# hyye/lio-mapping

Hardware: AMD Instinct MI355X
Metric: sliding-window solves/sec, 64-line 130k-pt scans, window=15 (opt_window=5) (higher is better)
Workload: dtype f64 (solve) / f32 (features); 1 GPU; HDL-64E outdoor_test_config_64, S_outdoor ray-cast scans, window_size=15 opt_window_size=5, one SolveOptimization per step, clouds resident in HBM; n_lidar_residuals=78236, local_map_points=76752, surf_stack_points=19386, parallelism=1 window

## Files before the change

lio-mapping_amd/csrc/cloud_device.h:

```cpp
#pragma once
#include <hip/hip_runtime.h>

#include <cfloat>
#include <climits>

#include "cloud_kernels.h"
#include "hmath.h"

#if defined(__HIPCC__)
namespace lio {

__device__ inline bool finite3(const float4 &p) { return isfinite(p.x) && isfinite(p.y) && isfinite(p.z); }
__device__ inline bool finite3(const Vec3<float> &p) { return isfinite(p.x) && isfinite(p.y) && isfinite(p.z); }


template <bool NORMALISE_CONJ>
__device__ __forceinline__ float4 to_end_point(float4 p, float s, const Quat<float> &qe, const Vec3<float> &te) {
  p.x -= s * te.x; p.y -= s * te.y; p.z -= s * te.z;
  Quat<float> qid;
  Quat<float> qs = slerp(qid, s, qe, FLT_EPSILON);
  Quat<float> qc = conj(qs);
  if (NORMALISE_CONJ) qc = normalized(qc);
  Vec3<float> v = rotate(qc, Vec3<float>(p.x, p.y, p.z));
  v = rotate(qe, v);
  p.x = v.x + te.x; p.y = v.y + te.y; p.z = v.z + te.z;
  return p;
}
__device__ __forceinline__ float4 rigid_map_point(float4 p, const Quat<float> &q, const Vec3<float> &t) {
  const Vec3<float> v = rotate(q, Vec3<float>(p.x, p.y, p.z));
  return make_float4(v.x + t.x, v.y + t.y, v.z + t.z, p.w);
}

__device__ inline int cell_coord(float v, float inv_cell) { return int(floorf(v * inv_cell)); }
__device__ __forceinline__ bool cell_of(float x, float y, float z, const GridDesc &g, int &cx, int &cy, int &cz) {
  cx = cell_coord(x, g.inv_cell) - g.origin[0];
  cy = cell_coord(y, g.inv_cell) - g.origin[1];
  cz = cell_coord(z, g.inv_cell) - g.origin[2];
  return cx >= 0 && cy >= 0 && cz >= 0 && cx < g.dims[0] && cy < g.dims[1] && cz < g.dims[2];
}
__device__ __forceinline__ uint32_t cell_index(int cx, int cy, int cz, const GridDesc &g) { return uint32_t(cx + g.dims[0] * (cy + g.dims[1] * cz)); }
__device__ __forceinline__ uint32_t cell_key_clamped(const float4 &p, const GridDesc &g) {
  int cx, cy, cz;
  cell_of(p.x, p.y, p.z, g, cx, cy, cz);
  cx = min(max(cx, 0), g.dims[0] - 1); cy = min(max(cy, 0), g.dims[1] - 1); cz = min(max(cz, 0), g.dims[2] - 1);
  return cell_index(cx, cy, cz, g);
}

__device__ __forceinline__ void cell_count_point(const float4 *__restrict__ pts, int i, const GridDesc &g, uint32_t *__restrict__ keys,
                                                 uint32_t *__restrict__ slot, int *__restrict__ cnt) {
  const uint32_t c = cell_key_clamped(pts[i], g);
  keys[i] = c;
  slot[i] = uint32_t(atomicAdd(&cnt[c], 1));
}
__device__ __forceinline__ void cell_place_point(const float4 *__restrict__ pts, const uint32_t *__restrict__ keys, const uint32_t *__restrict__ slot, int i,
                                                 const int *__restrict__ starts, float4 *__restrict__ sorted, int *__restrict__ cnt) {
  float4 p = pts[i];
  p.w = __int_as_float(i);
  const uint32_t c = keys[i];
  sorted[starts[c] + int(slot[i])] = p;
  cnt[c] = 0;
}

#define SEG_SCAN_THREADS 1024
#define SEG_SCAN_ITEMS 4
__device__ __forceinline__ void block_exclusive_scan(const int *__restrict__ in, int *__restrict__ out, int n, int base) {
  __shared__ int wsum[SEG_SCAN_THREADS / 64];
  const int tid = threadIdx.x, lane = tid & 63, wv = tid >> 6;
  int carry = base;
  for (int c0 = 0; c0 < n; c0 += SEG_SCAN_THREADS * SEG_SCAN_ITEMS) {
    const int i0 = c0 + tid * SEG_SCAN_ITEMS;
    int v[SEG_SCAN_ITEMS], tsum = 0;
#pragma unroll
    for (int k = 0; k < SEG_SCAN_ITEMS; ++k) { v[k] = i0 + k < n ? in[i0 + k] : 0; tsum += v[k]; }
    int inc = tsum;
#pragma unroll
    for (int off = 1; off < 64; off <<= 1) {
      const int u = __shfl_up(inc, off, 64);
      if (lane >= off) inc += u;
    }
    if (lane == 63) wsum[wv] = inc;
    __syncthreads();
    int before = 0, total = 0;
#pragma unroll
    for (int w = 0; w < SEG_SCAN_THREADS / 64; ++w) { const int t = wsum[w]; if (w < wv) before += t; total += t; }
    int run = carry + before + inc - tsum;
#pragma unroll
    for (int k = 0; k < SEG_SCAN_ITEMS; ++k)
      if (i0 + k < n) { out[i0 + k] = run; run += v[k]; }
    carry += total;
    __syncthreads();
  }
}

#define VOX_TILE 256
#define VOX_KEY_NONE 0xFFFFFFFFu

template <int ZBITS>
__device__ __forceinline__ bool vox_abs_key(const float4 &p, float inv_leaf, uint32_t &key) {
  constexpr int ZOFF = 1 << (ZBITS - 1);
  const float cx = floorf(p.x * inv_leaf), cy = floorf(p.y * inv_leaf), cz = floorf(p.z * inv_leaf);
  if (!(fabsf(cx) < 1024.f && fabsf(cy) < 1024.f && fabsf(cz) < float(ZOFF - 1))) return false;
  key = (uint32_t(int(cz) + ZOFF) << 22) | (uint32_t(int(cy) + 1024) << 11) | uint32_t(int(cx) + 1024);
  return true;
}

__device__ __forceinline__ void vox_block_partial(float (&mn)[3], float (&mx)[3], float cnt, float *__restrict__ row) {
  __shared__ float sm[7][VOX_TILE / 64];
  const int lane = threadIdx.x & 63, wv = threadIdx.x >> 6;
#pragma unroll
  for (int o = 32; o > 0; o >>= 1) {
    for (int d = 0; d < 3; ++d) { mn[d] = fminf(mn[d], __shfl_xor(mn[d], o, 64)); mx[d] = fmaxf(mx[d], __shfl_xor(mx[d], o, 64)); }
    cnt += __shfl_xor(cnt, o, 64);
  }
  if (lane == 0) { for (int d = 0; d < 3; ++d) { sm[d][wv] = mn[d]; sm[3 + d][wv] = mx[d]; } sm[6][wv] = cnt; }
  __syncthreads();
  if (threadIdx.x < 7) {
    const int t = threadIdx.x;
    float v = sm[t][0];
    for (int w = 1; w < VOX_TILE / 64; ++w) v = t < 3 ? fminf(v, sm[t][w]) : (t < 6 ? fmaxf(v, sm[t][w]) : v + sm[t][w]);
    row[t] = v;
  }
}

__device__ __forceinline__ bool vox_fold_bounds(const float *__restrict__ partial, int nb, float inv_leaf, VoxParams &v) {
  __shared__ float sm[7][VOX_TILE];
  const int t = threadIdx.x;
  float mn[3] = {FLT_MAX, FLT_MAX, FLT_MAX}, mx[3] = {-FLT_MAX, -FLT_MAX, -FLT_MAX};
  float cnt = 0;
  for (int b = t; b < nb; b += VOX_TILE) {
    for (int d = 0; d < 3; ++d) { mn[d] = fminf(mn[d], partial[size_t(b) * 8 + d]); mx[d] = fmaxf(mx[d], partial[size_t(b) * 8 + 3 + d]); }
    cnt += partial[size_t(b) * 8 + 6];
  }
  for (int d = 0; d < 3; ++d) { sm[d][t] = mn[d]; sm[3 + d][t] = mx[d]; }
  sm[6][t] = cnt;
  __syncthreads();
  for (int st = VOX_TILE / 2; st > 0; st >>= 1) {
    if (t < st) {
      for (int d = 0; d < 3; ++d) { sm[d][t] = fminf(sm[d][t], sm[d][t + st]); sm[3 + d][t] = fmaxf(sm[3 + d][t], sm[3 + d][t + st]); }
      sm[6][t] += sm[6][t + st];
    }
    __syncthreads();
  }
  if (t != 0) return false;
  long long dd[3];
  for (int d = 0; d < 3; ++d) {
    v.mn[d] = sm[d][0]; v.mx[d] = sm[3 + d][0];
    dd[d] = (long long)((v.mx[d] - v.mn[d]) * inv_leaf) + 1;
    v.minb[d] = int(floorf(v.mn[d] * inv_leaf));
    const int maxb = int(floorf(v.mx[d] * inv_leaf));
    v.divb[d] = maxb - v.minb[d] + 1;
  }
  v.overflow = (sm[6][0] > 0 && dd[0] * dd[1] * dd[2] > (long long)INT_MAX) ? 1 : 0;
  v.n_valid = int(sm[6][0]);
  return true;
}

__device__ __forceinline__ bool vox_is_head(const uint32_t *__restrict__ keys, int i, uint32_t k) {
  return k != VOX_KEY_NONE && (i == 0 || keys[i - 1] != k);
}
__device__ __forceinline__ void vox_tile_head_count(const uint32_t *__restrict__ keys, int n, int tile, int *__restrict__ count) {
  __shared__ int swave[VOX_TILE / 64];
  const int i = tile * VOX_TILE + threadIdx.x;
  const uint32_t k = i < n ? keys[i] : VOX_KEY_NONE;
  const unsigned long long b = __ballot(vox_is_head(keys, i, k));
  if ((threadIdx.x & 63) == 0) swave[threadIdx.x >> 6] = __popcll(b);
  __syncthreads();
  if (threadIdx.x == 0) *count = (swave[0] + swave[1]) + (swave[2] + swave[3]);
}

struct VoxSlot { int pos; bool head; };
__device__ __forceinline__ VoxSlot vox_centroid_tile(const float4 *__restrict__ pts, const uint32_t *__restrict__ keys, const uint32_t *__restrict__ vals,
                                                     const int *__restrict__ tile_heads, int n, int tile, float4 *__restrict__ out) {
  __shared__ float4 sp[VOX_TILE];
  __shared__ uint32_t sk[VOX_TILE];
  __shared__ int swave[VOX_TILE / 64], sbase[VOX_TILE / 64];
  const int tid = threadIdx.x, lane = tid & 63, wv = tid >> 6;
  const int base_i = tile * VOX_TILE, i = base_i + tid;
  int before = 0;
  for (int b = tid; b < tile; b += VOX_TILE) before += tile_heads[b];
#pragma unroll
  for (int o = 32; o > 0; o >>= 1) before += __shfl_xor(before, o, 64);
  const uint32_t k = i < n ? keys[i] : VOX_KEY_NONE;
  sk[tid] = k;
  if (k != VOX_KEY_NONE) sp[tid] = pts[vals[i]];
  const bool head = vox_is_head(keys, i, k);
  const unsigned long long hb = __ballot(head);
  if (lane == 0) { swave[wv] = __popcll(hb); sbase[wv] = before; }
  __syncthreads();
  int pos = (sbase[0] + sbase[1]) + (sbase[2] + sbase[3]);
  for (int w = 0; w < wv; ++w) pos += swave[w];
  pos += __popcll(hb & ((1ull << lane) - 1ull));
  if (head) {
    float ax = 0, ay = 0, az = 0, ai = 0;
    int e = tid;
    while (e < VOX_TILE && sk[e] == k) { const float4 p = sp[e]; ax += p.x; ay += p.y; az += p.z; ai += p.w; ++e; }
    int cnt = e - tid;
    if (e == VOX_TILE) {
      int g = base_i + VOX_TILE;
      while (g < n && keys[g] == k) { const float4 p = pts[vals[g]]; ax += p.x; ay += p.y; az += p.z; ai += p.w; ++g; ++cnt; }
    }
    const float c = float(cnt);
    out[pos] = make_float4(ax / c, ay / c, az / c, ai / c);
  }
  return VoxSlot{pos, head};
}

__device__ __forceinline__ void clear_valid_block(uint8_t *__restrict__ valid, size_t n) {
  const size_t i = (size_t(blockIdx.x) * VOX_TILE + threadIdx.x) * 16;
  if (i + 16 <= n) *reinterpret_cast<uint4 *>(valid + i) = make_uint4(0, 0, 0, 0);
  else for (size_t k = i; k < n; ++k) valid[k] = 0;
}
__device__ __forceinline__ void odom_state_init(OdomState *__restrict__ st, const float *__restrict__ T, bool converged) {
  static_assert(offsetof(OdomState, T) == 0 && sizeof(OdomState) <= VOX_TILE * 4, "state layout: T first, the rest zero");
  unsigned *o = reinterpret_cast<unsigned *>(st);
  const int nw = int(sizeof(OdomState) / 4);
  if (int(threadIdx.x) < nw) {
    unsigned v = threadIdx.x < 8 ? __float_as_uint(T[threadIdx.x]) : 0u;
    if (converged && threadIdx.x == offsetof(OdomState, converged) / 4) v = 1u;
    o[threadIdx.x] = v;
  }
}


#define FEAT_LPQ 8
#ifndef KNN_BATCH
#define KNN_BATCH 4
#endif
__device__ __forceinline__ unsigned long long knn_key(float d, int idx) {
  return (static_cast<unsigned long long>(__float_as_uint(d)) << 32) | static_cast<unsigned int>(idx);
}
template <int K>
__device__ __forceinline__ void knn_insert(unsigned long long key, int j, unsigned long long (&bk)[K], int (&bj)[K]) {
  if (key < bk[K - 1]) {
    bk[K - 1] = key; bj[K - 1] = j;
#pragma unroll
    for (int k = K - 1; k > 0; --k) {
      const bool sw = bk[k - 1] > bk[k];
      const unsigned long long tk = sw ? bk[k - 1] : bk[k];
      const int tj = sw ? bj[k - 1] : bj[k];
      bk[k - 1] = sw ? bk[k] : bk[k - 1];
      bj[k - 1] = sw ? bj[k] : bj[k - 1];
      bk[k] = tk; bj[k] = tj;
    }
  }
}
template <int K, int LPQ>
__device__ inline void knn_scan_group(const Vec3<float> &q, bool active, int sub, const float4 *__restrict__ map,
                                      const int *__restrict__ cells, const GridDesc &g, float (&bd)[K], int (&bi)[K], int (&bj)[K]) {
  unsigned long long bk[K];
#pragma unroll
  for (int k = 0; k < K; ++k) { bk[k] = knn_key(INFINITY, INT_MAX); bj[k] = 0; }
  int cx, cy, cz;
  cell_of(q.x, q.y, q.z, g, cx, cy, cz);
  if (!finite3(q) || cx < 0 || cy < 0 || cz < 0 || cx >= g.dims[0] || cy >= g.dims[1] || cz >= g.dims[2]) active = false;
  if (active) {
    const int x0 = max(cx - 1, 0), x1 = min(cx + 1, g.dims[0] - 1);
    if constexpr (LPQ <= 2) {
      const float uy = q.y * g.inv_cell, uz = q.z * g.inv_cell;
      const float fy = uy - floorf(uy), fz = uz - floorf(uz);
      const float cell = 1.0f / g.inv_cell;
      const float ey_lo = fmaxf(fy - 1e-3f, 0.f) * cell, ey_hi = fmaxf(1.0f - fy - 1e-3f, 0.f) * cell;
      const float ez_lo = fmaxf(fz - 1e-3f, 0.f) * cell, ez_hi = fmaxf(1.0f - fz - 1e-3f, 0.f) * cell;
      auto walk = [&](int j) {
        const float4 pc = map[j];
        float ddx = pc.x - q.x, ddy = pc.y - q.y, ddz = pc.z - q.z;
        float d = ddx * ddx;
        d += ddy * ddy;
        d += ddz * ddz;
        knn_insert<K>(knn_key(d, __float_as_int(pc.w)), j, bk, bj);
      };
      {
        const int row = g.dims[0] * (cy + g.dims[1] * cz);
        const int a = cells[row + x0], e = cells[row + x1 + 1];
        for (int j = a + sub; j < e; j += LPQ) walk(j);
      }
#pragma unroll
      for (int ph = 0; ph < 2; ++ph) {
        int s0 = 0, s1 = 0, s2 = 0, s3 = 0, c1 = 0, c2 = 0, c3 = 0, T = 0;
        const float worst = __uint_as_float(static_cast<unsigned int>(bk[K - 1] >> 32));
#pragma unroll
        for (int qq = 0; qq < 4; ++qq) {
          const int r = 1 + 4 * ph + qq;
          const int dy = int((0x22161u >> (2 * r)) & 3u) - 1, dz = int((0x28215u >> (2 * r)) & 3u) - 1;
          const int z = cz + dz, y = cy + dy;
          const float ey = dy < 0 ? ey_lo : (dy > 0 ? ey_hi : 0.f), ez = dz < 0 ? ez_lo : (dz > 0 ? ez_hi : 0.f);
          const bool on = z >= 0 && z < g.dims[2] && y >= 0 && y < g.dims[1] && !(ey * ey + ez * ez > worst);
          const int row = on ? g.dims[0] * (y + g.dims[1] * z) : 0;
          const int a = (on ? cells[row + x0] : 0) + sub, e = on ? cells[row + x1 + 1] : 0;
          const int len = e > a ? (e - a + LPQ - 1) / LPQ : 0;
          if (qq == 0) { s0 = a; c1 = len; }
          if (qq == 1) { s1 = a; c2 = c1 + len; }
          if (qq == 2) { s2 = a; c3 = c2 + len; }
          if (qq == 3) { s3 = a; T = c3 + len; }
        }
        for (int f = 0; f < T; ++f) {
          int j = s0 + f * LPQ;
          j = f >= c1 ? s1 + (f - c1) * LPQ : j;
          j = f >= c2 ? s2 + (f - c2) * LPQ : j;
          j = f >= c3 ? s3 + (f - c3) * LPQ : j;
          walk(j);
        }
      }
    } else {
      int rs[9], pre[10];
      pre[0] = 0;
#pragma unroll
      for (int r = 0; r < 9; ++r) {
        const int z = cz + r / 3 - 1, y = cy + r % 3 - 1;
        const bool in = z >= 0 && z < g.dims[2] && y >= 0 && y < g.dims[1];
        const int row = g.dims[0] * (y + g.dims[1] * z);
        const int a = in ? cells[row + x0] : 0, b = in ? cells[row + x1 + 1] : 0;
        rs[r] = a;
        pre[r + 1] = b - a;
      }
#pragma unroll
      for (int r = 0; r < 9; ++r) pre[r + 1] = pre[r] + max(pre[r + 1], 0);
      const int T = pre[9];
      for (int base = sub; base < T; base += LPQ * KNN_BATCH) {
        float4 p[KNN_BATCH];
        int jj[KNN_BATCH];
#pragma unroll
        for (int b = 0; b < KNN_BATCH; ++b) {
          const int f = base + b * LPQ;
          int j = f + rs[0];
#pragma unroll
          for (int r = 1; r < 9; ++r) j = f >= pre[r] ? f - pre[r] + rs[r] : j;
          jj[b] = f < T ? j : -1;
          p[b] = f < T ? map[j] : make_float4(0, 0, 0, 0);
        }
#pragma unroll
        for (int b = 0; b < KNN_BATCH; ++b) {
          if (jj[b] < 0) continue;
          float ddx = p[b].x - q.x, ddy = p[b].y - q.y, ddz = p[b].z - q.z;
          float d = ddx * ddx;
          d += ddy * ddy;
          d += ddz * ddz;
          knn_insert<K>(knn_key(d, __float_as_int(p[b].w)), jj[b], bk, bj);
        }
      }
    }
  }
#pragma unroll
  for (int m = 1; m < LPQ; m <<= 1) {
    unsigned long long ok[K]; int oj[K];
#pragma unroll
    for (int k = 0; k < K; ++k) {
      const unsigned int lo = __shfl_xor(static_cast<unsigned int>(bk[k]), m, 64), hi = __shfl_xor(static_cast<unsigned int>(bk[k] >> 32), m, 64);
      ok[k] = (static_cast<unsigned long long>(hi) << 32) | lo;
      oj[k] = __shfl_xor(bj[k], m, 64);
    }
#pragma unroll
    for (int c = 0; c < K; ++c) knn_insert<K>(ok[c], oj[c], bk, bj);
  }
#pragma unroll
  for (int k = 0; k < K; ++k) { bd[k] = __uint_as_float(static_cast<unsigned int>(bk[k] >> 32)); bi[k] = int(static_cast<unsigned int>(bk[k])); }
}

// ... 332 lines not shown
```

lio-mapping_amd/csrc/cloud_kernels.h:

```cpp
#pragma once
#include <cmath>
#include <cstdint>

#include "dev.h"

namespace lio {

struct VoxParams {
  float mn[3], mx[3];
  int minb[3], divb[3];
  int overflow;
  int n_valid;
};

struct Affine3f { float m[12]; };

#define LIO_MAX_FRAMES 32

struct ConcatSeg { const float4 *src; int n; int dst_off; int set_intensity; float intensity; Affine3f tf; int identity; };
struct ConcatArgs { ConcatSeg seg[LIO_MAX_FRAMES]; int nseg; int total; };
void launch_transform_concat(const ConcatArgs &a, float4 *dst, hipStream_t s);

void launch_deskew_to_end(float4 *pts, int n, const float q[4], const float p[3], float time_factor, hipStream_t s, bool keep_intensity = false);
void launch_rigid_map(const float4 *in, int n, const float q[4], const float p[3], float4 *out, hipStream_t s);

void launch_cloud_bounds(const float4 *pts, int n, DBuf<float> &partial, VoxParams *d_out, hipStream_t s);

class VoxelGridDev {
 public:
  size_t run(const float4 *in, size_t n, float leaf, DBuf<float4> &out, hipStream_t s, VoxParams *host_params = nullptr);
  void launch(const float4 *in, size_t n, float leaf, DBuf<float4> &out, hipStream_t s);
  size_t finish(VoxParams *host_params = nullptr);
  void set_host_signal(bool on) { use_signal_ = on; }
  VoxelGridDev() = default;
  VoxelGridDev(const VoxelGridDev &) = delete;
  VoxelGridDev &operator=(const VoxelGridDev &) = delete;

 private:
  const float4 *p_in_ = nullptr; size_t p_n_ = 0; DBuf<float4> *p_out_ = nullptr; hipStream_t p_stream_ = nullptr;
  float p_leaf_ = 0.f;
  void enqueue(bool exact);
  HostBuf<char> h_mail_;
  int *h_count_ = nullptr;
  VoxParams *h_params_ = nullptr;
  DBuf<float> partial_;
  DBuf<VoxParams> params_;
  DBuf<uint32_t> keys_, keys2_, vals_, vals2_;
  DBuf<int> count_, tile_heads_;
  DBuf<char> tmp_;
  unsigned *h_flag_ = nullptr;
  unsigned seq_ = 0;
  HostSignal sig_{};
  bool use_signal_ = true;
};

struct GridDesc {
  int origin[3];
  int dims[3];
  float inv_cell;
  int n_points;
};

inline float knn_cell_edge(float min_match_sq_dis) { return std::sqrt(min_match_sq_dis) * 1.0001f + 1e-6f; }
inline size_t grid_extent(GridDesc &g, const float mn[3], const float mx[3], float cell) {
  g.inv_cell = 1.0f / cell;
  size_t ncells = 1;
  for (int d = 0; d < 3; ++d) {
    const int lo = int(std::floor(mn[d] * g.inv_cell)) - 1, hi = int(std::floor(mx[d] * g.inv_cell)) + 1;
    g.origin[d] = lo; g.dims[d] = hi - lo + 1;
    ncells *= size_t(g.dims[d]);
  }
  return ncells;
}

class KnnGrid {
 public:
  void build(const float4 *pts, size_t n, const float mn[3], const float mx[3], float cell, hipStream_t s);
  const float4 *sorted() const { return sorted_.p; }
  const int *cells() const { return cells_.p; }
  const GridDesc &desc() const { return desc_; }

 private:
  GridDesc desc_{};
  DBuf<uint32_t> keys_, keys2_, vals_, vals2_;
  DBuf<float4> sorted_;
  DBuf<int> cells_, cnt_;
  bool cnt_dirty_ = false;
  DBuf<char> tmp_;
};

struct FeatFrame { const float4 *stack; int M; int slot_off; int tf_index; const uint32_t *order = nullptr; };
struct FeatArgs {
  FeatFrame fr[LIO_MAX_FRAMES];
  int nframes;
  int max_M;
  float min_match_sq_dis, min_plane_dis;
  int mapping_mode;
  float fixed_pz[3];
};
void launch_features(const FeatArgs &a, const float *transforms, const float4 *map_sorted, const int *cells, const GridDesc &g,
                     uint8_t *valid, float4 *coef, float *score, const int *skip_flag, hipStream_t s, float4 *abs_coef = nullptr);

void launch_knn(const float4 *query, int m, int k, float radius_sq, const float4 *map_sorted, const int *cells, const GridDesc &g,
                int32_t *idx, float *sqd, hipStream_t s);
void launch_knn_walk(const float4 *query, int m, int lanes_per_query, const float4 *map_sorted, const int *cells, const GridDesc &g,
                     int32_t *idx, float *sqd, float *nbr_xyz, hipStream_t s);

void launch_fit_five(int form, float min_match_sq_dis, float min_plane_dis, const float fixed_pz[3], const float *transform, const float4 *stack,
                     int m, const float4 *nbr, const float *fifth_sqd, uint8_t *valid, float4 *coef, float *score, float4 *abs_coef, hipStream_t s);

void launch_map_round(const FeatArgs &surf, const float4 *corner_stack, int Mc, const float *transform, const float4 *corner_map,
                      const int *corner_cells, const GridDesc &corner_grid, const float4 *surf_map, const int *surf_cells,
                      const GridDesc &surf_grid, uint8_t *valid, float4 *coef, float4 *abs_coef, const int *skip_flag, hipStream_t s);

struct SolveSetup {
  float tf[LIO_MAX_FRAMES][8];
  int ntf;
  float odom_T[8];
  int set_odom;
};
struct OdomState;
void launch_solve_setup(const SolveSetup &a, float *d_transforms, OdomState *d_odom, uint8_t *valid, size_t n_valid, hipStream_t s);

struct OdomState {
  float T[8];
  int converged;
  int iters;
  int degenerate;
  int kz;
  int nsel;
};
void launch_odom_rows(const float4 *stack, int M, int nslots, const uint8_t *valid, const float4 *coef, const OdomState *st,
                      double *partials, int nblocks, hipStream_t s, int b_from_coef = 0);
void launch_odom_update(const double *partials, int nblocks, OdomState *st, int iter, hipStream_t s, int min_rows = 0, int left_update = 0,
                        OdomState *mail = nullptr, const HostSignal &sig = HostSignal());
int odom_rows_blocks(int nslots);
int odom_round_blocks(int M, int lpq);
void launch_odom_round(const FeatArgs &a, int base_slot, int round, int keep, OdomState *st, const float4 *map_sorted, const int *cells, const GridDesc &g,
                       uint8_t *valid, float4 *coef, float *score, double *partials, hipStream_t s, OdomState *mail = nullptr,
                       const HostSignal &sig = HostSignal(), int lpq = 8);

void launch_gn_rows_map(const float4 *stack, int m, const uint8_t *valid, const float4 *coef, const OdomState *st, int b_from_coef, uint8_t *ok_out,
                        float *rows_out, hipStream_t s);
void launch_gn_fold(const double *partials, int nblocks, int wide, double *sums_out, hipStream_t s);
void launch_gn_step(const double *sums, OdomState *st, int iter, int min_rows, int left_update, hipStream_t s);

struct KfDesc {
  int slot_off, Mc, Ms;
  int map;
  int nb;
  int part_off;
  float pz[3];
};
struct KfMapDesc {
  const float4 *corner_sorted; const int *corner_cells; GridDesc corner_grid;
  const float4 *surf_sorted; const int *surf_cells; GridDesc surf_grid;
};
void launch_kf_query_keys(const KfDesc *kd, const KfMapDesc *md, const OdomState *st, int n_keyframes, int max_Mc, int max_Ms, const float4 *stack_all, uint32_t *keys,
                          hipStream_t s);
void launch_kf_round(const KfDesc *kd, const KfMapDesc *md, const OdomState *st, int n_keyframes, int max_Mc, int max_Ms, long long total_queries,
                     const float4 *stack_all, const uint32_t *order_or_null, float min_match_sq_dis, float min_plane_dis, int mapping_mode, uint8_t *valid, float4 *coef,
                     hipStream_t s);
void launch_kf_rows(const KfDesc *kd, const OdomState *st, int n_keyframes, int max_nb, const float4 *stack_all, const uint8_t *valid, const float4 *coef,
                    double *partials, int b_from_coef, hipStream_t s);
void launch_kf_update(const KfDesc *kd, OdomState *st, int n_keyframes, const double *partials, int iter, int min_rows, int left_update, int *n_converged,
                      hipStream_t s);

#if defined(__HIPCC__)
__device__ inline void reduce_partials28(const double *__restrict__ partials, int nblocks, double *ssum ) {
  __shared__ double part28[8][32];
  const int c = threadIdx.x & 31, g = threadIdx.x >> 5;
  double v = 0;
  if (c < 28 && g < 8)
    for (int b = g; b < nblocks; b += 8) v += partials[b * 28 + c];
  if (g < 8) part28[g][c] = v;
  __syncthreads();
  if (threadIdx.x < 28) {
    double s = 0;
#pragma unroll
    for (int k = 0; k < 8; ++k) s += part28[k][threadIdx.x];
    ssum[threadIdx.x] = s;
  }
  __syncthreads();
}
#endif

}
```

lio-mapping_amd/csrc/cloud_kernels.hip:

```cpp
#include <cstring>
#include <hip/hip_runtime.h>
#include <rocprim/rocprim.hpp>

#include <cfloat>
#include <climits>

#include "cloud_kernels.h"
#include "cloud_device.h"

namespace lio {

__global__ void k_transform_concat(ConcatArgs a, float4 *__restrict__ dst) {
  int gid = blockIdx.x * blockDim.x + threadIdx.x;
  if (gid >= a.total) return;
  int sidx = 0;
  for (int k = 1; k < a.nseg; ++k)
    if (gid >= a.seg[k].dst_off) sidx = k;
  const ConcatSeg &sg = a.seg[sidx];
  int local = gid - sg.dst_off;
  float4 p = sg.src[local];
  float4 o;
  if (sg.identity) {
    o = p;
  } else {
    const float *m = sg.tf.m;
    o.x = m[0] * p.x + m[1] * p.y + m[2] * p.z + m[3];
    o.y = m[4] * p.x + m[5] * p.y + m[6] * p.z + m[7];
    o.z = m[8] * p.x + m[9] * p.y + m[10] * p.z + m[11];
    o.w = p.w;
  }
  if (sg.set_intensity) o.w = sg.intensity;
  dst[gid] = o;
}

void launch_transform_concat(const ConcatArgs &a, float4 *dst, hipStream_t s) {
  if (a.total <= 0) return;
  hipLaunchKernelGGL(k_transform_concat, dim3(cdiv(a.total, 256)), dim3(256), 0, s, a, dst);
  LIO_HIP(hipGetLastError());
}

template <bool KEEP>
__global__ void __launch_bounds__(256) k_deskew_to_end(float4 *pts, int n, Quat<float> qe, Vec3<float> te, float time_factor) {
  int i = blockIdx.x * blockDim.x + threadIdx.x;
  if (i >= n) return;
  float4 p = pts[i];
  float s = time_factor * (p.w - int(p.w));
  if (!KEEP) p.w -= int(p.w);
  pts[i] = to_end_point<true>(p, s, qe, te);
}
void launch_deskew_to_end(float4 *pts, int n, const float q[4], const float p[3], float time_factor, hipStream_t s, bool keep_intensity) {
  if (n <= 0) return;
  const Quat<float> qe(q[3], q[0], q[1], q[2]);
  const Vec3<float> te(p[0], p[1], p[2]);
  if (keep_intensity) hipLaunchKernelGGL(k_deskew_to_end<true>, dim3(cdiv(n, 256)), dim3(256), 0, s, pts, n, qe, te, time_factor);
  else hipLaunchKernelGGL(k_deskew_to_end<false>, dim3(cdiv(n, 256)), dim3(256), 0, s, pts, n, qe, te, time_factor);
  LIO_HIP(hipGetLastError());
}

__global__ void __launch_bounds__(256) k_rigid_map(const float4 *__restrict__ in, int n, Quat<float> q, Vec3<float> t, float4 *__restrict__ out) {
  const int i = blockIdx.x * blockDim.x + threadIdx.x;
  if (i >= n) return;
  out[i] = rigid_map_point(in[i], q, t);
}
void launch_rigid_map(const float4 *in, int n, const float q[4], const float p[3], float4 *out, hipStream_t s) {
  if (n <= 0) return;
  hipLaunchKernelGGL(k_rigid_map, dim3(cdiv(n, 256)), dim3(256), 0, s, in, n, Quat<float>(q[3], q[0], q[1], q[2]), Vec3<float>(p[0], p[1], p[2]), out);
  LIO_HIP(hipGetLastError());
}

__global__ void k_bounds_partial(const float4 *__restrict__ pts, int n, float *__restrict__ partial) {
  float mn[3] = {FLT_MAX, FLT_MAX, FLT_MAX}, mx[3] = {-FLT_MAX, -FLT_MAX, -FLT_MAX};
  int cnt = 0;
  for (int i = blockIdx.x * blockDim.x + threadIdx.x; i < n; i += gridDim.x * blockDim.x) {
    float4 p = pts[i];
    if (!finite3(p)) continue;
    ++cnt;
    mn[0] = fminf(mn[0], p.x); mn[1] = fminf(mn[1], p.y); mn[2] = fminf(mn[2], p.z);
    mx[0] = fmaxf(mx[0], p.x); mx[1] = fmaxf(mx[1], p.y); mx[2] = fmaxf(mx[2], p.z);
  }
  __shared__ float sm[7][256];
  int t = threadIdx.x;
  for (int d = 0; d < 3; ++d) { sm[d][t] = mn[d]; sm[3 + d][t] = mx[d]; }
  sm[6][t] = float(cnt);
  __syncthreads();
  for (int st = 128; st > 0; st >>= 1) {
    if (t < st) {
      for (int d = 0; d < 3; ++d) { sm[d][t] = fminf(sm[d][t], sm[d][t + st]); sm[3 + d][t] = fmaxf(sm[3 + d][t], sm[3 + d][t + st]); }
      sm[6][t] += sm[6][t + st];
    }
    __syncthreads();
  }
  if (t < 7) partial[blockIdx.x * 8 + t] = sm[t][0];
}

__global__ void __launch_bounds__(256) k_bounds_final(const float *__restrict__ partial, int nb, float inv_leaf, VoxParams *out) {
  VoxParams v;
  if (vox_fold_bounds(partial, nb, inv_leaf, v)) *out = v;
}

__global__ void k_vox_keys(const float4 *__restrict__ pts, int n, float inv_leaf, const VoxParams *__restrict__ vp,
                           uint32_t *__restrict__ keys, uint32_t *__restrict__ vals) {
  int i = blockIdx.x * blockDim.x + threadIdx.x;
  if (i >= n) return;
  float4 p = pts[i];
  uint32_t key = VOX_KEY_NONE;
  if (finite3(p)) {
    int i0 = int(floorf(p.x * inv_leaf) - float(vp->minb[0]));
    int i1 = int(floorf(p.y * inv_leaf) - float(vp->minb[1]));
    int i2 = int(floorf(p.z * inv_leaf) - float(vp->minb[2]));
    key = uint32_t(i0 + i1 * vp->divb[0] + i2 * vp->divb[0] * vp->divb[1]);
  }
  keys[i] = key;
  vals[i] = uint32_t(i);
}

__global__ void __launch_bounds__(VOX_TILE) k_vox_keys_abs(const float4 *__restrict__ pts, int n, float inv_leaf, uint32_t *__restrict__ keys,
                                                          uint32_t *__restrict__ vals, float *__restrict__ partial, int *__restrict__ range_overflow) {
  const int i = blockIdx.x * VOX_TILE + threadIdx.x;
  float mn[3] = {FLT_MAX, FLT_MAX, FLT_MAX}, mx[3] = {-FLT_MAX, -FLT_MAX, -FLT_MAX};
  float cnt = 0;
  if (i < n) {
    const float4 p = pts[i];
    uint32_t key = VOX_KEY_NONE;
    if (finite3(p)) {
      cnt = 1.f;
      mn[0] = mx[0] = p.x; mn[1] = mx[1] = p.y; mn[2] = mx[2] = p.z;
      if (!vox_abs_key<10>(p, inv_leaf, key)) *range_overflow = 1;
    }
    keys[i] = key;
    vals[i] = uint32_t(i);
  }
  vox_block_partial(mn, mx, cnt, partial + size_t(blockIdx.x) * 8);
}

__global__ void __launch_bounds__(VOX_TILE) k_vox_tile_heads(const uint32_t *__restrict__ keys, int n, int *__restrict__ tile_heads,
                                                             const float *__restrict__ partial, int npartial, float inv_leaf, VoxParams *__restrict__ params) {
  if (blockIdx.x == gridDim.x - 1) {
    if (npartial <= 0) return;
    VoxParams v;
    if (vox_fold_bounds(partial, npartial, inv_leaf, v)) *params = v;
    return;
  }
  vox_tile_head_count(keys, n, blockIdx.x, tile_heads + blockIdx.x);
}

struct VoxMail { int count; VoxParams params; int range_overflow; };
__global__ void __launch_bounds__(VOX_TILE) k_vox_centroids(const float4 *__restrict__ pts, const uint32_t *__restrict__ keys,
                                                            const uint32_t *__restrict__ vals, const int *__restrict__ tile_heads, int n,
                                                            float4 *__restrict__ out, int *__restrict__ count, const VoxParams *__restrict__ params,
                                                            int *__restrict__ range_overflow, VoxMail *mail, HostSignal sig) {
  const VoxSlot r = vox_centroid_tile(pts, keys, vals, tile_heads, n, blockIdx.x, out);
  if (blockIdx.x == gridDim.x - 1) {
    __shared__ VoxMail smail;
    const int tid = threadIdx.x;
    if (tid == VOX_TILE - 1) {
      const int total = r.pos + (r.head ? 1 : 0);
      *count = total;
      smail.count = total; smail.params = *params; smail.range_overflow = *range_overflow;
      if (sig.flag) *range_overflow = 0;
    }
    if (sig.flag) {
      __syncthreads();
      if (tid < 64) post_host_mail(sig, mail, &smail, int(sizeof(VoxMail) / 4), tid);
    }
  }
}

void launch_cloud_bounds(const float4 *pts, int n, DBuf<float> &partial, VoxParams *d_out, hipStream_t s) {
  const int nb = std::max(1, std::min(cdiv(n, 256), 512));
  partial.reserve(size_t(nb) * 8);
  hipLaunchKernelGGL(k_bounds_partial, dim3(nb), dim3(256), 0, s, pts, n, partial.p);
  hipLaunchKernelGGL(k_bounds_final, dim3(1), dim3(256), 0, s, partial.p, nb, 1.0f, d_out);
  LIO_HIP(hipGetLastError());
}

void VoxelGridDev::launch(const float4 *in, size_t n, float leaf, DBuf<float4> &out, hipStream_t s) {
  p_in_ = in; p_n_ = n; p_out_ = &out; p_stream_ = s; p_leaf_ = leaf;
  if (n == 0) return;
  enqueue(false);
}

void VoxelGridDev::enqueue(bool exact) {
  const float4 *in = p_in_;
  const size_t n = p_n_;
  DBuf<float4> &out = *p_out_;
  hipStream_t s = p_stream_;
  const int ni = int(n);
  const float inv_leaf = 1.0f / p_leaf_;
  const int nkb = cdiv(ni, VOX_TILE);
  partial_.reserve(size_t(std::max(nkb, 512)) * 8);
  params_.reserve(1);
  keys_.reserve(n); keys2_.reserve(n); vals_.reserve(n); vals2_.reserve(n);
  if (count_.cap < 2) { count_.reserve(2); LIO_HIP(hipMemsetAsync(count_.p, 0, count_.cap * sizeof(int), s)); }
  out.reserve(n);
  if (!h_count_) {
    h_mail_.alloc(256, hipHostMallocCoherent, true);
    static_assert(sizeof(VoxMail) <= 128, "mailbox layout");
    h_count_ = reinterpret_cast<int *>(h_mail_.p);
    h_params_ = reinterpret_cast<VoxParams *>(h_count_ + 1);
    h_flag_ = reinterpret_cast<unsigned *>(reinterpret_cast<char *>(h_count_) + 128);
  }
  int *d_range = count_.p + 1;
  if (!use_signal_) LIO_HIP(hipMemsetAsync(d_range, 0, sizeof(int), s));
  int npartial = 0;
  if (exact) {
    const int nb = std::min(cdiv(ni, 256), 512);
    hipLaunchKernelGGL(k_bounds_partial, dim3(nb), dim3(256), 0, s, in, ni, partial_.p);
    hipLaunchKernelGGL(k_bounds_final, dim3(1), dim3(256), 0, s, partial_.p, nb, inv_leaf, params_.p);
    hipLaunchKernelGGL(k_vox_keys, dim3(cdiv(ni, 256)), dim3(256), 0, s, in, ni, inv_leaf, params_.p, keys_.p, vals_.p);
  } else {
    hipLaunchKernelGGL(k_vox_keys_abs, dim3(nkb), dim3(VOX_TILE), 0, s, in, ni, inv_leaf, keys_.p, vals_.p, partial_.p, d_range);
    npartial = nkb;
  }
  size_t tmp_bytes = 0;
  LIO_HIP(rocprim::radix_sort_pairs(nullptr, tmp_bytes, keys_.p, keys2_.p, vals_.p, vals2_.p, n, 0, 32, s));
  tmp_.reserve(tmp_bytes + 256);
  LIO_HIP(rocprim::radix_sort_pairs(tmp_.p, tmp_bytes, keys_.p, keys2_.p, vals_.p, vals2_.p, n, 0, 32, s));
  const int ntiles = cdiv(ni, VOX_TILE);
  tile_heads_.reserve(ntiles);
  hipLaunchKernelGGL(k_vox_tile_heads, dim3(ntiles + 1), dim3(VOX_TILE), 0, s, keys2_.p, ni, tile_heads_.p, partial_.p, npartial, inv_leaf, params_.p);
  sig_ = HostSignal();
  if (use_signal_) { sig_.flag = h_flag_; sig_.seq = ++seq_; }

  hipLaunchKernelGGL(k_vox_centroids, dim3(ntiles), dim3(VOX_TILE), 0, s, in, keys2_.p, vals2_.p, tile_heads_.p, ni, out.p, count_.p, params_.p, d_range,
                     reinterpret_cast<VoxMail *>(h_count_), sig_);
  LIO_HIP(hipGetLastError());
  if (!sig_.flag) {
    VoxMail *m = reinterpret_cast<VoxMail *>(h_count_);
    LIO_HIP(hipMemcpyAsync(&m->count, count_.p, sizeof(int), hipMemcpyDeviceToHost, s));
    LIO_HIP(hipMemcpyAsync(&m->params, params_.p, sizeof(VoxParams), hipMemcpyDeviceToHost, s));
    LIO_HIP(hipMemcpyAsync(&m->range_overflow, d_range, sizeof(int), hipMemcpyDeviceToHost, s));
  }
}

size_t VoxelGridDev::finish(VoxParams *host_params) {
  if (p_n_ == 0) {
    if (host_params) std::memset(host_params, 0, sizeof(*host_params));
    return 0;
  }
  const VoxMail *m = reinterpret_cast<const VoxMail *>(h_count_);
  bool redone = false;
  for (;;) {
    if (sig_.flag) wait_host_signal(sig_, p_stream_);
    else LIO_HIP(hipStreamSynchronize(p_stream_));
    if (m->range_overflow == 1 && !redone) {
      enqueue(true);
      redone = true;
      continue;
    }
    if (redone) LIO_HIP(hipStreamSynchronize(p_stream_));
    break;
  }
  int count = m->count;
  const VoxParams hp = m->params;
  if (hp.overflow) {
    p_out_->reserve(p_n_);
    LIO_HIP(hipMemcpyAsync(p_out_->p, p_in_, p_n_ * sizeof(float4), hipMemcpyDeviceToDevice, p_stream_));
    LIO_HIP(hipStreamSynchronize(p_stream_));
    count = int(p_n_);
  }
  if (host_params) *host_params = hp;
  return size_t(count);
}

size_t VoxelGridDev::run(const float4 *in, size_t n, float leaf, DBuf<float4> &out, hipStream_t s, VoxParams *host_params) {
  launch(in, n, leaf, out, s);
  return finish(host_params);
}

__global__ void k_cell_count(const float4 *__restrict__ pts, int n, GridDesc g, uint32_t *__restrict__ keys, uint32_t *__restrict__ slot,
                             int *__restrict__ cnt) {
  int i = blockIdx.x * blockDim.x + threadIdx.x;
  if (i >= n) return;
  cell_count_point(pts, i, g, keys, slot, cnt);
}

__global__ void k_cell_place(const float4 *__restrict__ pts, const uint32_t *__restrict__ keys, const uint32_t *__restrict__ slot, int n,
                             const int *__restrict__ starts, float4 *__restrict__ sorted, int *__restrict__ cnt) {
  int i = blockIdx.x * blockDim.x + threadIdx.x;
  if (i >= n) return;
  cell_place_point(pts, keys, slot, i, starts, sorted, cnt);
}

void KnnGrid::build(const float4 *pts, size_t n, const float mn[3], const float mx[3], float cell, hipStream_t s) {
  desc_.n_points = int(n);
  const size_t ncells = grid_extent(desc_, mn, mx, cell);
  if (ncells > (size_t(1) << 30)) throw DeviceError("KnnGrid: cell table too large");
  cells_.reserve(ncells + 1);
  if (cnt_.cap < ncells + 1 || cnt_dirty_) {
    cnt_.reserve(ncells + 1);
    LIO_HIP(hipMemsetAsync(cnt_.p, 0, cnt_.cap * sizeof(int), s));
  }
  cnt_dirty_ = true;
  keys_.reserve(std::max<size_t>(n, 1)); vals_.reserve(std::max<size_t>(n, 1)); sorted_.reserve(std::max<size_t>(n, 1));
  const int ni = int(n);
  if (ni) hipLaunchKernelGGL(k_cell_count, dim3(cdiv(ni, 256)), dim3(256), 0, s, pts, ni, desc_, keys_.p, vals_.p, cnt_.p);
  size_t tmp_bytes = 0;
  LIO_HIP(rocprim::exclusive_scan(nullptr, tmp_bytes, cnt_.p, cells_.p, 0, ncells + 1, rocprim::plus<int>(), s));
  tmp_.reserve(tmp_bytes + 256);
  LIO_HIP(rocprim::exclusive_scan(tmp_.p, tmp_bytes, cnt_.p, cells_.p, 0, ncells + 1, rocprim::plus<int>(), s));
  if (ni) hipLaunchKernelGGL(k_cell_place, dim3(cdiv(ni, 256)), dim3(256), 0, s, pts, keys_.p, vals_.p, ni, cells_.p, sorted_.p, cnt_.p);
  LIO_HIP(hipGetLastError());
  cnt_dirty_ = false;
}

#define KNN_WALK_THREADS 256
template <int K, int LPQ>
__global__ void __launch_bounds__(KNN_WALK_THREADS) k_nn_walk(const float4 *__restrict__ query, int m, int cut, float radius_sq,
                                                              const float4 *__restrict__ map, const int *__restrict__ cells, GridDesc g,
                                                              int32_t *__restrict__ idx, float *__restrict__ sqd, float *__restrict__ nbr) {
  const int gt = blockIdx.x * blockDim.x + threadIdx.x;
  const int i = gt / LPQ, sub = gt % LPQ;
  const bool active = i < m;
  const float4 q4 = active ? query[i] : make_float4(0, 0, 0, 0);
  float bd[K]; int bi[K], bj[K];
  knn_scan_group<K, LPQ>(Vec3<float>(q4.x, q4.y, q4.z), active, sub, map, cells, g, bd, bi, bj);
  if (!active || sub != 0) return;
#pragma unroll
  for (int k = 0; k < K; ++k) {
    const bool ok = bi[k] != INT_MAX && !(cut && !(bd[k] < radius_sq));
    const size_t o = size_t(i) * K + k;
    idx[o] = ok ? bi[k] : -1;
    sqd[o] = ok ? bd[k] : INFINITY;
    if (nbr) {
      const float4 p = ok ? map[bj[k]] : make_float4(0, 0, 0, 0);
      nbr[3 * o + 0] = p.x; nbr[3 * o + 1] = p.y; nbr[3 * o + 2] = p.z;
    }
  }
}

template <int K, int LPQ>
static void launch_knn_walk_as(const float4 *query, int m, int cut, float radius_sq, const float4 *map_sorted, const int *cells, const GridDesc &g,
                               int32_t *idx, float *sqd, float *nbr, hipStream_t s) {
  hipLaunchKernelGGL((k_nn_walk<K, LPQ>), dim3(cdiv((long long)m * LPQ, KNN_WALK_THREADS)), dim3(KNN_WALK_THREADS), 0, s, query, m, cut, radius_sq,
                     map_sorted, cells, g, idx, sqd, nbr);
}

void launch_knn(const float4 *query, int m, int k, float radius_sq, const float4 *map_sorted, const int *cells, const GridDesc &g,
                int32_t *idx, float *sqd, hipStream_t s) {
  if (m <= 0) return;
  if (k == 1) launch_knn_walk_as<1, 8>(query, m, 1, radius_sq, map_sorted, cells, g, idx, sqd, nullptr, s);
  else if (k == 5) launch_knn_walk_as<5, 8>(query, m, 1, radius_sq, map_sorted, cells, g, idx, sqd, nullptr, s);
  else throw DeviceError("launch_knn: k is 1 or 5");
  LIO_HIP(hipGetLastError());
}

void launch_knn_walk(const float4 *query, int m, int lanes_per_query, const float4 *map_sorted, const int *cells, const GridDesc &g,
                     int32_t *idx, float *sqd, float *nbr_xyz, hipStream_t s) {
  if (m <= 0) return;
  if (lanes_per_query == 1) launch_knn_walk_as<5, 1>(query, m, 0, 0.f, map_sorted, cells, g, idx, sqd, nbr_xyz, s);
  else if (lanes_per_query == 4) launch_knn_walk_as<5, 4>(query, m, 0, 0.f, map_sorted, cells, g, idx, sqd, nbr_xyz, s);
  else if (lanes_per_query == 8) launch_knn_walk_as<5, 8>(query, m, 0, 0.f, map_sorted, cells, g, idx, sqd, nbr_xyz, s);
  else throw DeviceError("launch_knn_walk: lanes per query is 1, 4 or 8");
  LIO_HIP(hipGetLastError());
}

template <bool MAPPING, int LPQ>
__global__ void __launch_bounds__(FEAT_THREADS) k_features(FeatArgs a, const float *__restrict__ transforms, const float4 *__restrict__ map,
                                                          const int *__restrict__ cells, GridDesc g, uint8_t *__restrict__ valid,
                                                          float4 *__restrict__ coef, float *__restrict__ score, const int *__restrict__ skip_flag,
                                                          float4 *__restrict__ abs_coef) {
  if (skip_flag && *skip_flag) return;
  features_block<MAPPING, LPQ>(a.fr[blockIdx.y], feat_scalars(a), int(blockIdx.x), transforms, map, cells, g, valid, coef, score, abs_coef);
}

__device__ __forceinline__ uint8_t line_features_fit(const Vec3<float> &t, const Vec3<float> &pz, const Vec3<float> &sel, float min_match_sq_dis,
                                                     float bd4, int bi4, const int (&bj)[5], const float4 *__restrict__ map, float4 &c) {
  uint8_t ok = 0;
  c = make_float4(0, 0, 0, 0);
  if (bi4 != INT_MAX && bd4 < min_match_sq_dis) {
// ... 410 lines not shown
```

Measured before the change: 2174 solves/s.

## Replace device radix sort with block tile sort plus rank-merge for small voxel clouds

```diff
diff --git a/lio-mapping_amd/csrc/cloud_device.h b/lio-mapping_amd/csrc/cloud_device.h
--- a/lio-mapping_amd/csrc/cloud_device.h
+++ b/lio-mapping_amd/csrc/cloud_device.h
@@ -1,11 +1,13 @@
 #pragma once
 #include <hip/hip_runtime.h>
+#include <rocprim/block/block_radix_sort.hpp>
 
 #include <cfloat>
 #include <climits>
 
 #include "cloud_kernels.h"
 #include "hmath.h"
+#include "vox_rank.h"
 
 #if defined(__HIPCC__)
 namespace lio {
@@ -104,8 +106,9 @@
   return true;
 }
 
+template <int THREADS = VOX_TILE>
 __device__ __forceinline__ void vox_block_partial(float (&mn)[3], float (&mx)[3], float cnt, float *__restrict__ row) {
-  __shared__ float sm[7][VOX_TILE / 64];
+  __shared__ float sm[7][THREADS / 64];
   const int lane = threadIdx.x & 63, wv = threadIdx.x >> 6;
 #pragma unroll
   for (int o = 32; o > 0; o >>= 1) {
@@ -117,7 +120,7 @@
   if (threadIdx.x < 7) {
     const int t = threadIdx.x;
     float v = sm[t][0];
-    for (int w = 1; w < VOX_TILE / 64; ++w) v = t < 3 ? fminf(v, sm[t][w]) : (t < 6 ? fmaxf(v, sm[t][w]) : v + sm[t][w]);
+    for (int w = 1; w < THREADS / 64; ++w) v = t < 3 ? fminf(v, sm[t][w]) : (t < 6 ? fmaxf(v, sm[t][w]) : v + sm[t][w]);
     row[t] = v;
   }
 }
@@ -203,6 +206,136 @@
     out[pos] = make_float4(ax / c, ay / c, az / c, ai / c);
   }
   return VoxSlot{pos, head};
+}
+
+#define VOX_SORT_THREADS 1024
+#define VOX_SORT_ITEMS (VOX_SORT_TILE / VOX_SORT_THREADS)
+template <bool FUSED>
+__device__ __forceinline__ void vox_tile_sort_block(const float4 *__restrict__ pts, const uint32_t *keys_in, int n, int tile, float inv_leaf,
+                                                    uint32_t *keys_out, uint32_t *__restrict__ vals_out, uint32_t *__restrict__ samples,
+                                                    float *__restrict__ partial_row, int *__restrict__ range_overflow) {
+  using Sort = rocprim::block_radix_sort<uint32_t, VOX_SORT_THREADS, VOX_SORT_ITEMS, uint32_t>;
+  __shared__ typename Sort::storage_type ssort;
+  __shared__ uint32_t sk[VOX_SORT_TILE];
+  const int tid = threadIdx.x, base = tile * VOX_SORT_TILE;
+  float mn[3] = {FLT_MAX, FLT_MAX, FLT_MAX}, mx[3] = {-FLT_MAX, -FLT_MAX, -FLT_MAX};
+  float cnt = 0;
+#pragma unroll
+  for (int j = 0; j < VOX_SORT_ITEMS; ++j) {
+    const int p = j * VOX_SORT_THREADS + tid, i = base + p;
+    uint32_t key = VOX_KEY_NONE;
+    if (i < n) {
+      if (FUSED) {
+        const float4 pt = pts[i];
+        if (finite3(pt)) {
+          cnt += 1.f;
+          mn[0] = fminf(mn[0], pt.x); mn[1] = fminf(mn[1], pt.y); mn[2] = fminf(mn[2], pt.z);
+          mx[0] = fmaxf(mx[0], pt.x); mx[1] = fmaxf(mx[1], pt.y); mx[2] = fmaxf(mx[2], pt.z);
+          if (!vox_abs_key<10>(pt, inv_leaf, key)) *range_overflow = 1;
+        }
+      } else {
+        key = keys_in[i];
+      }
+    }
+    sk[p] = key;
+  }
+  __syncthreads();
+  uint32_t k[VOX_SORT_ITEMS], v[VOX_SORT_ITEMS];
+#pragma unroll
+  for (int j = 0; j < VOX_SORT_ITEMS; ++j) {
+    const int p = tid * VOX_SORT_ITEMS + j;
+    k[j] = sk[p];
+    v[j] = base + p < n ? uint32_t(base + p) : 0xFFFFFFFFu;
+  }
+  if (FUSED) vox_block_partial<VOX_SORT_THREADS>(mn, mx, cnt, partial_row);
+  Sort().sort_to_striped(k, v, ssort);
+#pragma unroll
+  for (int j = 0; j < VOX_SORT_ITEMS; ++j) {
+    const int p = j * VOX_SORT_THREADS + tid, i = base + p;
+    if (i < n) {
+      keys_out[i] = k[j];
+      vals_out[i] = v[j];
+      if ((p & (VOX_SORT_STRIDE - 1)) == 0) samples[size_t(tile) * VOX_SORT_SAMPLES + p / VOX_SORT_STRIDE] = k[j];
+    }
+  }
+}
+
+#define VOX_RANK_BATCH 8
+__device__ __forceinline__ void vox_rank_merge_block(const uint32_t *__restrict__ keys, const uint32_t *__restrict__ vals,
+                                                     const uint32_t *__restrict__ samples, int n, int block, uint32_t *__restrict__ keys2,
+                                                     uint32_t *__restrict__ vals2) {
+  static_assert(VOX_SORT_SAMPLES % 4 == 0 && VOX_RANK_WINDOW == 128, "the table is copied four words at a time; a lane stages two keys of a window");
+  __shared__ uint4 ssamp4[VOX_RANK_MAX_N / VOX_SORT_STRIDE / 4];
+  __shared__ int sbr[VOX_TILE / 64][2][VOX_RANK_MAX_TILES];
+  __shared__ uint32_t swin[VOX_TILE / 64][VOX_RANK_BATCH][VOX_RANK_WINDOW];
+  const uint32_t *ssamp = reinterpret_cast<const uint32_t *>(ssamp4);
+  const int tid = threadIdx.x, lane = tid & 63, wv = tid >> 6;
+  const int ntiles = vox_sort_tiles(n);
+  for (int j = tid; j < ntiles * (VOX_SORT_SAMPLES / 4); j += VOX_TILE) ssamp4[j] = reinterpret_cast<const uint4 *>(samples)[j];
+  const int gw = block * (VOX_TILE / 64) + wv;
+  const int tile = min(gw / VOX_RANK_TILE_GROUPS, ntiles - 1);
+  const int tlen = vox_sort_tile_len(n, tile), w = vox_rank_group(tlen);
+  const int first = (gw - tile * VOX_RANK_TILE_GROUPS) * w;
+  const int cnt = min(w, tlen - first);
+  const bool wave_on = cnt > 0, mine = lane < cnt;
+  const int i = tile * VOX_SORT_TILE + first + lane;
+  const uint32_t k = mine ? keys[i] : VOX_KEY_NONE;
+  const uint32_t kmin = __shfl(k, 0, 64), kmax = __shfl(k, wave_on ? cnt - 1 : 0, 64);
+  __syncthreads();
+  if (wave_on) {
+    for (int r = lane; r < ntiles; r += 64) {
+      if (r == tile) continue;
+      const uint32_t *ts = ssamp + r * VOX_SORT_SAMPLES, *tk = keys + size_t(r) * VOX_SORT_TILE;
+      const int len = vox_sort_tile_len(n, r);
+      sbr[wv][0][r] = vox_tile_bound(ts, tk, len, kmin, r < tile);
+      sbr[wv][1][r] = vox_tile_bound(ts, tk, len, kmax, r < tile);
+    }
+  }
+  __syncthreads();
+  if (!wave_on) return;
+  bool all_lo, all_up;
+  const uint32_t front_lo = vox_front_key(k, false, all_lo), front_up = vox_front_key(k, true, all_up);
+  int dest = first + lane;
+  for (int r0 = 0; r0 < ntiles; r0 += VOX_RANK_BATCH) {
+    int lo[VOX_RANK_BATCH], hi[VOX_RANK_BATCH], pos[VOX_RANK_BATCH];
+    uint32_t e0[VOX_RANK_BATCH], e1[VOX_RANK_BATCH], front[VOX_RANK_BATCH];
+#pragma unroll
+    for (int b = 0; b < VOX_RANK_BATCH; ++b) {
+      const int r = r0 + b;
+      const bool on = r < ntiles && r != tile;
+      lo[b] = on ? sbr[wv][0][r] : 0;
+      hi[b] = on ? sbr[wv][1][r] : 0;
+      const uint32_t *tk = keys + size_t(r) * VOX_SORT_TILE + lo[b] + lane;
+      e0[b] = lo[b] + lane < hi[b] ? tk[0] : VOX_KEY_NONE;
+      e1[b] = lo[b] + 64 + lane < hi[b] ? tk[64] : VOX_KEY_NONE;
+      front[b] = r < tile ? front_up : front_lo;
+    }
+    __builtin_amdgcn_fence(__ATOMIC_RELEASE, "wavefront");
+    __builtin_amdgcn_wave_barrier();
+#pragma unroll
+    for (int b = 0; b < VOX_RANK_BATCH; ++b) { swin[wv][b][lane] = e0[b]; swin[wv][b][64 + lane] = e1[b]; }
+    __builtin_amdgcn_fence(__ATOMIC_RELEASE, "wavefront");
+    __builtin_amdgcn_wave_barrier();
+    __builtin_amdgcn_fence(__ATOMIC_ACQUIRE, "wavefront");
+    const uint32_t(*win)[VOX_RANK_WINDOW] = swin[wv];
+    vox_count_windows<VOX_RANK_WINDOW, VOX_RANK_BATCH>([win](int b, int j) { return win[b][j]; }, front, pos);
+#pragma unroll
+    for (int b = 0; b < VOX_RANK_BATCH; ++b) {
+      const int r = r0 + b;
+      const int len = hi[b] - lo[b];
+      const bool all = r < tile && all_up;
+      dest += lo[b] + (all ? len : min(pos[b], min(len, VOX_RANK_WINDOW)));
+      for (int c = lo[b] + VOX_RANK_WINDOW; c < hi[b] && !all; c += VOX_RANK_WINDOW) {
+        const uint32_t *tk = keys + size_t(r) * VOX_SORT_TILE + c;
+        const int m = min(VOX_RANK_WINDOW, hi[b] - c);
+        const uint32_t f1[1] = {front[b]};
+        int p1[1];
+        vox_count_windows<VOX_RANK_WINDOW, 1>([tk, m](int, int j) { return j < m ? tk[j] : VOX_KEY_NONE; }, f1, p1);
+        dest += p1[0];
+      }
+    }
+  }
+  if (mine && unsigned(dest) < unsigned(n)) { keys2[dest] = k; vals2[dest] = vals[i]; }
 }
 
 __device__ __forceinline__ void clear_valid_block(uint8_t *__restrict__ valid, size_t n) {
diff --git a/lio-mapping_amd/csrc/cloud_kernels.h b/lio-mapping_amd/csrc/cloud_kernels.h
--- a/lio-mapping_amd/csrc/cloud_kernels.h
+++ b/lio-mapping_amd/csrc/cloud_kernels.h
@@ -46,6 +46,7 @@
   DBuf<float> partial_;
   DBuf<VoxParams> params_;
   DBuf<uint32_t> keys_, keys2_, vals_, vals2_;
+  DBuf<uint32_t> samples_;
   DBuf<int> count_, tile_heads_;
   DBuf<char> tmp_;
   unsigned *h_flag_ = nullptr;
diff --git a/lio-mapping_amd/csrc/cloud_kernels.hip b/lio-mapping_amd/csrc/cloud_kernels.hip
--- a/lio-mapping_amd/csrc/cloud_kernels.hip
+++ b/lio-mapping_amd/csrc/cloud_kernels.hip
@@ -133,6 +133,18 @@
   vox_block_partial(mn, mx, cnt, partial + size_t(blockIdx.x) * 8);
 }
 
+template <bool FUSED>
+__global__ void __launch_bounds__(VOX_SORT_THREADS) k_vox_tile_sort(const float4 *__restrict__ pts, const uint32_t *keys_in, int n, float inv_leaf, uint32_t *keys_out,
+                                                           uint32_t *__restrict__ vals_out, uint32_t *__restrict__ samples, float *__restrict__ partial,
+                                                           int *__restrict__ range_overflow) {
+  vox_tile_sort_block<FUSED>(pts, keys_in, n, blockIdx.x, inv_leaf, keys_out, vals_out, samples, partial + size_t(blockIdx.x) * 8, range_overflow);
+}
+__global__ void __launch_bounds__(VOX_TILE) k_vox_rank_merge(const uint32_t *__restrict__ keys, const uint32_t *__restrict__ vals,
+                                                            const uint32_t *__restrict__ samples, int n, uint32_t *__restrict__ keys2,
+                                                            uint32_t *__restrict__ vals2) {
+  vox_rank_merge_block(keys, vals, samples, n, blockIdx.x, keys2, vals2);
+}
+
 __global__ void __launch_bounds__(VOX_TILE) k_vox_tile_heads(const uint32_t *__restrict__ keys, int n, int *__restrict__ tile_heads,
                                                              const float *__restrict__ partial, int npartial, float inv_leaf, VoxParams *__restrict__ params) {
   if (blockIdx.x == gridDim.x - 1) {
@@ -190,7 +202,8 @@
   const int nkb = cdiv(ni, VOX_TILE);
   partial_.reserve(size_t(std::max(nkb, 512)) * 8);
   params_.reserve(1);
-  keys_.reserve(n); keys2_.reserve(n); vals_.reserve(n); vals2_.reserve(n);
+  keys_.reserve((n + 3) & ~size_t(3));
+  keys2_.reserve(n); vals_.reserve(n); vals2_.reserve(n);
   if (count_.cap < 2) { count_.reserve(2); LIO_HIP(hipMemsetAsync(count_.p, 0, count_.cap * sizeof(int), s)); }
   out.reserve(n);
   if (!h_count_) {
@@ -203,19 +216,33 @@
   int *d_range = count_.p + 1;
   if (!use_signal_) LIO_HIP(hipMemsetAsync(d_range, 0, sizeof(int), s));
   int npartial = 0;
+  const bool small = n <= size_t(VOX_RANK_MAX_N);
   if (exact) {
     const int nb = std::min(cdiv(ni, 256), 512);
     hipLaunchKernelGGL(k_bounds_partial, dim3(nb), dim3(256), 0, s, in, ni, partial_.p);
     hipLaunchKernelGGL(k_bounds_final, dim3(1), dim3(256), 0, s, partial_.p, nb, inv_leaf, params_.p);
     hipLaunchKernelGGL(k_vox_keys, dim3(cdiv(ni, 256)), dim3(256), 0, s, in, ni, inv_leaf, params_.p, keys_.p, vals_.p);
-  } else {
+  } else if (!small) {
     hipLaunchKernelGGL(k_vox_keys_abs, dim3(nkb), dim3(VOX_TILE), 0, s, in, ni, inv_leaf, keys_.p, vals_.p, partial_.p, d_range);
     npartial = nkb;
   }
-  size_t tmp_bytes = 0;
-  LIO_HIP(rocprim::radix_sort_pairs(nullptr, tmp_bytes, keys_.p, keys2_.p, vals_.p, vals2_.p, n, 0, 32, s));
-  tmp_.reserve(tmp_bytes + 256);
-  LIO_HIP(rocprim::radix_sort_pairs(tmp_.p, tmp_bytes, keys_.p, keys2_.p, vals_.p, vals2_.p, n, 0, 32, s));
+  if (small) {
+    const int nst = vox_sort_tiles(ni);
+    samples_.reserve(size_t(nst) * VOX_SORT_SAMPLES);
+    uint32_t *ko = nst == 1 ? keys2_.p : keys_.p, *vo = nst == 1 ? vals2_.p : vals_.p;
+    if (exact) {
+      hipLaunchKernelGGL(k_vox_tile_sort<false>, dim3(nst), dim3(VOX_SORT_THREADS), 0, s, in, keys_.p, ni, inv_leaf, ko, vo, samples_.p, partial_.p, d_range);
+    } else {
+      hipLaunchKernelGGL(k_vox_tile_sort<true>, dim3(nst), dim3(VOX_SORT_THREADS), 0, s, in, nullptr, ni, inv_leaf, ko, vo, samples_.p, partial_.p, d_range);
+      npartial = nst;
+    }
+    if (nst > 1) hipLaunchKernelGGL(k_vox_rank_merge, dim3(cdiv(vox_rank_total_groups(ni), VOX_TILE / 64)), dim3(VOX_TILE), 0, s, keys_.p, vals_.p, samples_.p, ni, keys2_.p, vals2_.p);
+  } else {
+    size_t tmp_bytes = 0;
+    LIO_HIP(rocprim::radix_sort_pairs(nullptr, tmp_bytes, keys_.p, keys2_.p, vals_.p, vals2_.p, n, 0, 32, s));
+    tmp_.reserve(tmp_bytes + 256);
+    LIO_HIP(rocprim::radix_sort_pairs(tmp_.p, tmp_bytes, keys_.p, keys2_.p, vals_.p, vals2_.p, n, 0, 32, s));
+  }
   const int ntiles = cdiv(ni, VOX_TILE);
   tile_heads_.reserve(ntiles);
   hipLaunchKernelGGL(k_vox_tile_heads, dim3(ntiles + 1), dim3(VOX_TILE), 0, s, keys2_.p, ni, tile_heads_.p, partial_.p, npartial, inv_leaf, params_.p);
diff --git a/lio-mapping_amd/csrc/vox_rank.h b/lio-mapping_amd/csrc/vox_rank.h
--- /dev/null
+++ b/lio-mapping_amd/csrc/vox_rank.h
@@ -0,0 +1,89 @@
+#pragma once
+#include <cstddef>
+#include <cstdint>
+
+#if defined(__HIPCC__)
+#define VOX_HD __host__ __device__ __forceinline__
+#else
+#define VOX_HD inline
+#endif
+
+#define VOX_SORT_TILE 4096
+#define VOX_SORT_STRIDE 32
+#define VOX_RANK_MAX_N 262144
+#define VOX_SORT_SAMPLES (VOX_SORT_TILE / VOX_SORT_STRIDE)
+#define VOX_RANK_MAX_TILES (VOX_RANK_MAX_N / VOX_SORT_TILE)
+#define VOX_RANK_WINDOW 128
+
+static_assert(VOX_SORT_TILE % VOX_SORT_STRIDE == 0 && VOX_RANK_MAX_N % VOX_SORT_TILE == 0, "tiles hold whole strides, the cap whole tiles");
+static_assert(VOX_SORT_STRIDE % 4 == 0 && (VOX_SORT_SAMPLES & (VOX_SORT_SAMPLES - 1)) == 0, "a stride is whole 16-byte loads; the sample search halves its step");
+static_assert(VOX_RANK_MAX_N / VOX_SORT_STRIDE * 4 <= 64 * 1024, "the sample table is static LDS");
+
+namespace lio {
+
+VOX_HD int vox_sort_tiles(int n) { return (n + VOX_SORT_TILE - 1) / VOX_SORT_TILE; }
+VOX_HD int vox_sort_tile_len(int n, int tile) { const int r = n - tile * VOX_SORT_TILE; return r < VOX_SORT_TILE ? r : VOX_SORT_TILE; }
+
+VOX_HD uint32_t vox_front_key(uint32_t k, bool upper, bool &all) {
+  all = upper && k == 0xFFFFFFFFu;
+  return upper && !all ? k + 1u : k;
+}
+
+struct alignas(16) VoxKey4 { uint32_t v[4]; } __attribute__((may_alias));
+
+VOX_HD int vox_tile_bound(const uint32_t *samples, const uint32_t *tile_keys, int len, uint32_t k, bool upper) {
+  bool all;
+  const uint32_t front = vox_front_key(k, upper, all);
+  if (all) return len;
+  const int ns = (len + VOX_SORT_STRIDE - 1) / VOX_SORT_STRIDE;
+  int c = 0;
+  for (int s = VOX_SORT_SAMPLES; s > 0; s >>= 1) {
+    const int p = c + s;
+    if (p <= ns && samples[p - 1] < front) c = p;
+  }
+  if (c == 0) return 0;
+  const int base = (c - 1) * VOX_SORT_STRIDE;
+  const VoxKey4 *b4 = reinterpret_cast<const VoxKey4 *>(tile_keys + base);
+  int q = 0;
+#if defined(__HIPCC__)
+#pragma unroll
+#endif
+  for (int j = 0; j < VOX_SORT_STRIDE / 4; ++j) {
+    if (base + 4 * j < len) {
+      const VoxKey4 g = b4[j];
+      for (int t = 0; t < 4; ++t) q += (base + 4 * j + t < len && g.v[t] < front) ? 1 : 0;
+    }
+  }
+  return base + q;
+}
+
+#define VOX_RANK_TILE_GROUPS (VOX_SORT_TILE / 64)
+VOX_HD int vox_rank_group(int len) { const int w = len / VOX_RANK_TILE_GROUPS; return w < 1 ? 1 : w; }
+VOX_HD int vox_rank_groups(int len) { const int w = vox_rank_group(len); return (len + w - 1) / w; }
+VOX_HD int vox_rank_total_groups(int n) {
+  const int last = vox_sort_tiles(n) - 1;
+  return last * VOX_RANK_TILE_GROUPS + vox_rank_groups(vox_sort_tile_len(n, last));
+}
+
+VOX_HD int vox_rank_dest(const uint32_t *keys, const uint32_t *samples, int n, int tile, int i_in_tile, uint32_t k) {
+  int dest = i_in_tile;
+  const int ntiles = vox_sort_tiles(n);
+  for (int r = 0; r < ntiles; ++r) {
+    if (r == tile) continue;
+    dest += vox_tile_bound(samples + size_t(r) * VOX_SORT_SAMPLES, keys + size_t(r) * VOX_SORT_TILE, vox_sort_tile_len(n, r), k, r < tile);
+  }
+  return dest;
+}
+
+template <int W, int B, class Fetch>
+VOX_HD void vox_count_windows(Fetch fetch, const uint32_t (&front)[B], int (&pos)[B]) {
+  static_assert((W & (W - 1)) == 0, "the step halves");
+  for (int b = 0; b < B; ++b) pos[b] = 0;
+  for (int s = W / 2; s > 0; s >>= 1)
+    for (int b = 0; b < B; ++b)
+      if (fetch(b, pos[b] + s - 1) < front[b]) pos[b] += s;
+  for (int b = 0; b < B; ++b)
+    if (fetch(b, pos[b]) < front[b]) pos[b] += 1;
+}
+
+}
```

New measurement: 1027 solves/s. -52.7%, worse.
